# microsoft/timewarp

Hardware: AMD Instinct MI355X
Metric: MH-accepted samples/sec (whole node), alanine-dipeptide kernel_transformer_nvp (higher is better)
Workload: dtype f16x3 (split-fp16 operands, 3 MFMAs per fp32 product, fp32 accumulate)

## Files before the change

### timewarp_amd/csrc/tw_netblock_h3.hip

```cpp
#include <utility>
#include <vector>

#include "tw_common.h"

namespace tw {

typedef float f4 __attribute__((ext_vector_type(4)));
typedef _Float16 h8 __attribute__((ext_vector_type(8)));
typedef _Float16 h4 __attribute__((ext_vector_type(4)));
typedef unsigned u4 __attribute__((ext_vector_type(4)));
typedef unsigned u2 __attribute__((ext_vector_type(2)));

#define H3_NT 3
#define H3_FFN_SPLIT 4
#define H3_TOK (16 * H3_NT)
#define H3_XT 48
#define H3_XT_IMG 1536
#define H3_PAIR_BYTES 2048
#define H3_STAGE_PAIRS 4
#define H3_STAGE_TILE_BYTES 8192
#define H3_STAGE_BYTES 9216
#define H3_RING 5
#define H3_XT_BYTES (128 * H3_XT * 2)
#define H3_WAVE_LDS (2 * H3_XT_BYTES)
// ... 488 lines not shown
      for (int m = 0; m < V; ++m) row[m] = row[m] / den;
  }
  __syncthreads();
  char* out = sfrag + blockIdx.z * variant_bytes + blk * (int64_t)4 * H * ((int64_t)NG * nt * 2048);
  const bool paired = nt == H3N4_NT;
  for (int i = t; i < 4 * NG * nt * 64; i += nthr) {
    const int lane = i & 63, rest = i >> 6;
    const int jt = rest % nt, gi = (rest / nt) % NG, w = rest / (nt * NG);
    const int tq = 16 * nt * w + 16 * jt + (lane & 15);
    const int mq = tq / P, aq = tq - mq * P;
    const bool qok = mq < mpwg && aq < V;
    const float* row = E + (int64_t)(qok ? mq * V + aq : 0) * V;
    const int k0 = 16 * (win.w[w] / 32 + 2 * gi) + 8 * (lane >> 4);
    h8 hi, lo;
#pragma unroll
    for (int e = 0; e < 8; ++e) {
      const int tk = paired ? mq * P + 32 * gi + 4 * (lane >> 4) + (e < 4 ? e : e + 12) : k0 + e;
      const int ak = tk - mq * P;
      const float val = (qok && ak >= 0 && ak < V) ? row[ak] : 0.f;
      const _Float16 hh = (_Float16)val;
      hi[e] = hh;
      lo[e] = (_Float16)(val - (float)hh);
    }
    char* base = out + ((int64_t)(w * H + h) * (NG * nt) + (paired ? jt * NG + gi : gi * nt + jt)) * 2048;
    *(h8*)(base + lane * 16) = hi;
    *(h8*)(base + 1024 + lane * 16) = lo;
  }
}

struct H3Params {
  const char* packed;
  int64_t net_stride_bytes;
  int64_t stages;
  int64_t side_in2b, side_layers, side_layer_size, side_out2b, side_scales;
  const float* emb;
  const int32_t* types;
  const float* xc;
  const float* xv;
  const float* z_other;
  const char* sfrag;
  int sfrag_shared;
  int64_t sf_variant_bytes;
  int windowed;
  const float* rff;
  int d_rff;
  int win[4];
  float* out[2];
  float* dump;
  int64_t n_rows, n_cond;
  int V, mpw, nblocks;
  int ng;
  int P;
  int H, n_layers, ff_chunks, hid_chunks, d_emb;
  float eps;
  int net_sel;
  int debug;
  const uint8_t* masked;
  PrevCoupling prev;
};
__device__ __forceinline__ void h3_load_sf4(const char* p, u4 (&r)[16]) {
  asm volatile(
      "global_load_dwordx4 %0, %16, off\n\t"
      "global_load_dwordx4 %1, %16, off offset:1024\n\t"
      "global_load_dwordx4 %2, %16, off offset:2048\n\t"
      "global_load_dwordx4 %3, %16, off offset:3072\n\t"
      "global_load_dwordx4 %4, %17, off\n\t"
      "global_load_dwordx4 %5, %17, off offset:1024\n\t"
      "global_load_dwordx4 %6, %17, off offset:2048\n\t"
      "global_load_dwordx4 %7, %17, off offset:3072\n\t"
      "global_load_dwordx4 %8, %18, off\n\t"
      "global_load_dwordx4 %9, %18, off offset:1024\n\t"
      "global_load_dwordx4 %10, %18, off offset:2048\n\t"
      "global_load_dwordx4 %11, %18, off offset:3072\n\t"
      "global_load_dwordx4 %12, %19, off\n\t"
      "global_load_dwordx4 %13, %19, off offset:1024\n\t"
      "global_load_dwordx4 %14, %19, off offset:2048\n\t"
      "global_load_dwordx4 %15, %19, off offset:3072\n\t"
      "s_waitcnt vmcnt(0)"
      : "=&v"(r[0]), "=&v"(r[1]), "=&v"(r[2]), "=&v"(r[3]), "=&v"(r[4]), "=&v"(r[5]), "=&v"(r[6]), "=&v"(r[7]), "=&v"(r[8]),
        "=&v"(r[9]), "=&v"(r[10]), "=&v"(r[11]), "=&v"(r[12]), "=&v"(r[13]), "=&v"(r[14]), "=&v"(r[15])
      : "v"(p), "v"(p + H3N4_SF_BYTES), "v"(p + 2 * H3N4_SF_BYTES), "v"(p + 3 * H3N4_SF_BYTES)
      : "memory");
}

template <int NT>
struct BOp {
  h8 h[NT], l[NT];
};

__device__ __forceinline__ f4 mfma32(h8 a, h8 b, f4 c) { return __builtin_amdgcn_mfma_f32_16x16x32_f16(a, b, c, 0, 0, 0); }
__device__ __forceinline__ f4 mfma16(h4 a, h4 b, f4 c) { return __builtin_amdgcn_mfma_f32_16x16x16f16(a, b, c, 0, 0, 0); }

template <int NT>
__device__ __forceinline__ void mma3(const h8 ah, const h8 al, const BOp<NT>& b, f4 (&acc)[NT]) {
#pragma unroll
  for (int jt = 0; jt < NT; ++jt) acc[jt] = mfma32(ah, b.h[jt], acc[jt]);
#pragma unroll
  for (int jt = 0; jt < NT; ++jt) acc[jt] = mfma32(ah, b.l[jt], acc[jt]);
#pragma unroll
  for (int jt = 0; jt < NT; ++jt) acc[jt] = mfma32(al, b.h[jt], acc[jt]);
}

__device__ __forceinline__ void split_pair(float a, float b, unsigned& hi, unsigned& lo) {
  float ta, tb;
  asm("v_cvt_pk_f16_f32 %0, %4, %5\n\t"
      "v_fma_mix_f32 %2, %0, -1.0, %4 op_sel_hi:[1,0,0]\n\t"
// ... 58 lines not shown
      "global_load_dwordx4 %1, %12, off offset:1024\n\t"
      "global_load_dwordx2 %2, %13, off offset:2048\n\t"
      "global_load_dwordx2 %3, %13, off offset:2056\n\t"
      "global_load_dwordx4 %4, %14, off\n\t"
      "global_load_dwordx4 %5, %14, off offset:1024\n\t"
      "global_load_dwordx2 %6, %15, off offset:2048\n\t"
      "global_load_dwordx2 %7, %15, off offset:2056\n\t"
      "global_load_dwordx4 %8, %16, off\n\t"
      "global_load_dwordx4 %9, %16, off offset:1024\n\t"
      "global_load_dwordx2 %10, %17, off offset:2048\n\t"
      "global_load_dwordx2 %11, %17, off offset:2056\n\t"
      "s_waitcnt vmcnt(0)"
      : "=&v"(a[0]), "=&v"(b[0]), "=&v"(c[0]), "=&v"(d[0]), "=&v"(a[1]), "=&v"(b[1]), "=&v"(c[1]), "=&v"(d[1]),
        "=&v"(a[2]), "=&v"(b[2]), "=&v"(c[2]), "=&v"(d[2])
      : "v"(p16), "v"(p8), "v"(p16 + H3_SF_BYTES), "v"(p8 + H3_SF_BYTES), "v"(p16 + 2 * H3_SF_BYTES),
        "v"(p8 + 2 * H3_SF_BYTES)
      : "memory");
}



template <int NT>
__device__ __forceinline__ void h3_add_layernorm(f4 (&x)[8][NT], const f4 (&y)[8][NT], const float* lnw_lane,
                                                 const float* lnb_lane, float eps) {
  f4 w[8], b[8];
#pragma unroll
  for (int ft = 0; ft < 8; ++ft) {
    w[ft] = *(const f4*)(lnw_lane + 16 * ft);
    b[ft] = *(const f4*)(lnb_lane + 16 * ft);
  }
#pragma unroll
  for (int jt = 0; jt < NT; ++jt) {
    float s = 0.f;
#pragma unroll
    for (int ft = 0; ft < 8; ++ft) {
      x[ft][jt] = x[ft][jt] + y[ft][jt];
      s += (x[ft][jt][0] + x[ft][jt][1]) + (x[ft][jt][2] + x[ft][jt][3]);
    }
    const float mean = h3_xor_sum(s) * (1.f / 128.f);
    float q = 0.f;
#pragma unroll
    for (int ft = 0; ft < 8; ++ft) {
      x[ft][jt] = x[ft][jt] - mean;
      q += (x[ft][jt][0] * x[ft][jt][0] + x[ft][jt][1] * x[ft][jt][1]) +
           (x[ft][jt][2] * x[ft][jt][2] + x[ft][jt][3] * x[ft][jt][3]);
    }
    const float var = h3_xor_sum(q) * (1.f / 128.f);
    const float rstd = 1.0f / sqrtf(var + eps);
#pragma unroll
    for (int ft = 0; ft < 8; ++ft) x[ft][jt] = x[ft][jt] * rstd * w[ft] + b[ft];
  }
}

struct H3Pipe {
  const char* gnext;
  char* lds;
  int cur;
  int wave;
  int debug;
  int ring = H3_RING;

  __device__ __forceinline__ void fetch(int slot) {
    char* dst = lds + slot * H3_STAGE_BYTES;
#pragma unroll
    for (int i = 0; i < 2; ++i)
      __builtin_amdgcn_global_load_lds((const __attribute__((address_space(1))) void*)(gnext + wave * 2048 + i * 1024),
                                       (__attribute__((address_space(3))) void*)(dst + wave * 2048 + i * 1024), 16, 0, 0);
    if (wave == 0)
      __builtin_amdgcn_global_load_lds((const __attribute__((address_space(1))) void*)(gnext + H3_STAGE_TILE_BYTES),
                                       (__attribute__((address_space(3))) void*)(dst + H3_STAGE_TILE_BYTES), 16, 0, 0);
    gnext += H3_STAGE_BYTES;
  }
  __device__ __forceinline__ void start_issue() {
#pragma unroll
    for (int i = 0; i < H3_RING; ++i)
      if (i < ring) fetch(i);
    cur = 0;
  }
  __device__ __forceinline__ void start_wait() {
    asm volatile("s_waitcnt vmcnt(0)" ::: "memory");
    __builtin_amdgcn_s_barrier();
    asm volatile("" ::: "memory");
  }
  __device__ __forceinline__ const char* stage() const { return lds + cur * H3_STAGE_BYTES; }
  __device__ __forceinline__ void advance() {
    asm volatile("s_waitcnt vmcnt(0) lgkmcnt(0)" ::: "memory");
    if (!TW_EXPERIMENT(debug & TW_DEBUG_EXP_NO_BARRIERS)) __builtin_amdgcn_s_barrier();
    asm volatile("" ::: "memory");
    const int released = cur;
    cur = (cur + 1 == ring) ? 0 : cur + 1;
    if (!TW_EXPERIMENT(debug & TW_DEBUG_EXP_NO_WEIGHT_DMA)) fetch(released);
  }
};

struct H3Tiles {
  h8 t[2 * H3_STAGE_PAIRS];
  const char* base;
  __device__ __forceinline__ void rd(int p) {
    t[2 * p] = *(const h8*)(base + p * H3_PAIR_BYTES);
    t[2 * p + 1] = *(const h8*)(base + p * H3_PAIR_BYTES + 1024);
  }
  __device__ __forceinline__ void load(const char* st, int lane) {
    base = st + lane * 16;
    rd(0);
    rd(1);
    __builtin_amdgcn_sched_barrier(0);
// ... 114 lines not shown

template <int NT, bool ASM, bool DENSE = false, bool WIDE = false, bool RFF = false, bool ENC = false, bool H1 = false, bool NG6 = false>
__global__ void __launch_bounds__(256) __attribute__((amdgpu_waves_per_eu(1, 1)))
netblock_h3_kernel(const H3Params p) {
  extern __shared__ __attribute__((aligned(16))) char lds[];
  static_assert(!H1 || ENC || WIDE || (DENSE && ASM && !RFF) || (NT == 4 && ASM),
                "the single-MFMA variant exists as the encoder-stack build (<= 48 atoms), for the wide layout, and - MLP sections "
                "only, the softmax attention block stays in split form - for the dense model");
  static_assert(!WIDE || (ASM && !DENSE), "the wide layout exists for the asm build of the kernel-attention variant");
  static_assert(!NG6 || WIDE, "six-group windows belong to the wide layout");
  static_assert(!RFF || DENSE, "position features belong to the dense model");
  static_assert(!ENC || ASM, "the encoder-stack statement embeds the generated asm sections");
  static_assert(NT == 3 || (NT == 4 && !RFF && (!WIDE || (ENC && !NG6)) && (!DENSE || (ASM && !WIDE && !H1))),
                "64-token waves: the kernel-attention variant - one molecule of 49-64 atoms per wave, or (WIDE: the paired layout, "
                "encoder-stack statement only) one of 97-128 atoms per pair of waves; the dense softmax model on one molecule of "
                "49-64 atoms per wave: the encoder-stack statement (r06, tools/gen_h3_enc_asm.py --dense --nt=4), or the per-section "
                "build with its attention block compiled C++ (r05; activation dumps, section stamps)");
  constexpr int KIN = RFF ? 6 : 2;
  constexpr bool ASM_IO = ASM, ASM_ATT = ASM && !(DENSE && NT == 4);
  constexpr bool R6 = H3_R6(NT, DENSE, WIDE, RFF, ENC, H1);
  constexpr int RING = NT == 4 ? H3N4_RING : (R6 ? H3_RING + 1 : H3_RING);
  constexpr int XT_IMG = NT == 4 ? H3N4_XT_IMG : H3_XT_IMG;
  constexpr int SF_BYTES = NT == 4 ? H3N4_SF_BYTES : H3_SF_BYTES;
  constexpr int WAVE_LDS = NT == 4 ? H3N4_WAVE_LDS : (DENSE ? H3D_WAVE_LDS : (WIDE ? H3W_WAVE_LDS : H3_WAVE_LDS));
  constexpr int SIDE_LDS_OFFSET = NT == 4 ? H3N4_SIDE_LDS_OFFSET
                                          : (DENSE ? H3D_SIDE_LDS_OFFSET : (WIDE ? H3W_SIDE_LDS_OFFSET
                                                                                  : H3_SIDE_LDS_OFFSET + (R6 ? H3_STAGE_BYTES : 0)));
  constexpr int SIDE_CHUNKS = DENSE ? 5 : 3;
  const int wave = __builtin_amdgcn_readfirstlane(threadIdx.x >> 6);
  const int lane = threadIdx.x & 63;
  const int g = lane >> 4, i16 = lane & 15;

  int net, wg;
  if (p.net_sel < 0) {
    const int xcd = blockIdx.x & 7;
    net = xcd >> 2;
    wg = (blockIdx.x >> 3) * 4 + (xcd & 3);
  } else {
    net = p.net_sel;
    wg = blockIdx.x;
  }
  const int blk = wg * 4 + wave;
  const bool active = WIDE ? true : blk < p.nblocks;
  if (WIDE ? wg >= p.nblocks : wg * 4 >= p.nblocks) return;
  const int64_t row0 = (WIDE ? (int64_t)wg : (int64_t)blk) * p.mpw;
  const int slot0 = WIDE ? 16 * NT * wave : 0;

  const char* net_base = p.packed + (int64_t)net * p.net_stride_bytes;
  const float* side = (const float*)(net_base + p.stages * H3_STAGE_BYTES);
  const float* scales = side + p.side_scales;
  _Float16* xt_hi = (_Float16*)(lds + RING * H3_STAGE_BYTES + wave * WAVE_LDS);

  const unsigned long long t_kernel_top = (p.debug & TW_DEBUG_SECTION_STAMPS) ? __builtin_readcyclecounter() : 0ull;
  H3Pipe pipe;
  pipe.gnext = net_base + lane * 16;
  pipe.lds = lds;
  pipe.cur = 0;
  pipe.wave = wave;
  pipe.debug = p.debug;
  pipe.ring = RING;
  if constexpr (ENC && DENSE && NT == 3) {
    if (wave == 0) {
      const char* src = (const char*)(side + p.side_layers) + lane * 16;
      char* dst = lds + SIDE_LDS_OFFSET;
#pragma unroll
      for (int i = 0; i < SIDE_CHUNKS; ++i)
        __builtin_amdgcn_global_load_lds((const __attribute__((address_space(1))) void*)(src + i * 1024),
                                         (__attribute__((address_space(3))) void*)(dst + i * 1024), 16, 0, 0);
    }
  }
  pipe.start_issue();

  const float sc_in2 = scales[1], sc_out2 = scales[2 + 3 * p.n_layers + 1];
  f4 bb_in2[8];
#pragma unroll
  for (int ot = 0; ot < 8; ++ot) bb_in2[ot] = *(const f4*)(side + p.side_in2b + 4 * g + 16 * ot);
  const f4 bb_out2 = *(const f4*)(side + p.side_out2b + 4 * g);

  int64_t tok_row[NT];
  int64_t tok_cond[NT];
  int tok_atom[NT];
  const unsigned inv_v = (65536u + (unsigned)p.P - 1u) / (unsigned)p.P;
  const bool cond_shared = p.n_cond == 1, cond_per_row = p.n_cond >= p.n_rows;
#pragma unroll
  for (int jt = 0; jt < NT; ++jt) {
    const int t = slot0 + 16 * jt + i16;
    const int q = (int)(((unsigned)t * inv_v) >> 16);
    const int64_t n = row0 + q;
    const int atom = t - q * p.P;
    const bool ok = active && q < p.mpw && n < p.n_rows && atom < p.V;
    tok_row[jt] = ok ? n : -1;
    tok_cond[jt] = !ok || cond_shared ? 0 : (cond_per_row ? n : n % p.n_cond);
    tok_atom[jt] = ok ? atom : 0;
  }
  float zo[NT][3];
  {
    float part[NT];
    bool bad = false;
#pragma unroll
    for (int jt = 0; jt < NT; ++jt) {
      const int64_t n = tok_row[jt];
      part[jt] = 0.f;
#pragma unroll
      for (int k = 0; k < 3; ++k) zo[jt][k] = 0.f;
      if (n < 0) continue;
      const int64_t idx = (n * p.V + tok_atom[jt]) * 3;
      if (p.prev.s_raw) {
        float ld = 0.f;
#pragma unroll
        for (int k = 0; k < 3; ++k) {
          const float sr = p.prev.s_raw[idx + k], shift = p.prev.t[idx + k];
          const float scale = expf(sr);
          bad |= !(isfinite(sr) && isfinite(shift));
          const float z = p.prev.z_in[idx + k];
          zo[jt][k] = p.prev.reverse ? (z - shift) / scale : z * scale + shift;
          ld += logf(scale);
        }
        part[jt] = p.masked[tok_cond[jt] * p.V + tok_atom[jt]] ? 0.f : ld;
        if (net == 0 && g == 0) {
#pragma unroll
          for (int k = 0; k < 3; ++k) p.prev.z_out[idx + k] = zo[jt][k];
        }
      } else {
#pragma unroll
        for (int k = 0; k < 3; ++k) zo[jt][k] = p.z_other[idx + k];
      }
    }
    if constexpr (WIDE) {
      if (p.prev.s_raw) {
        float* scr = (float*)(lds + RING * H3_STAGE_BYTES);
        if (net == 0) {
          if (bad) atomicOr(p.prev.nonfinite, 1);
          if (g == 0) {
#pragma unroll
            for (int jt = 0; jt < NT; ++jt) scr[slot0 + 16 * jt + i16] = part[jt];
          }
        }
        asm volatile("s_waitcnt lgkmcnt(0)" ::: "memory");
        __builtin_amdgcn_s_barrier();
        if (net == 0 && wave == 0 && lane < p.mpw) {
          const int64_t n = row0 + lane;
          if (n < p.n_rows) {
            float acc = 0.f;
            for (int a = 0; a < p.V; ++a) acc += scr[lane * p.P + a];
            p.prev.delta_logp[n] -= p.prev.reverse ? -acc : acc;
          }
        }
        asm volatile("s_waitcnt lgkmcnt(0)" ::: "memory");
        __builtin_amdgcn_s_barrier();
      }
    } else
    if (p.prev.s_raw && net == 0) {
      if (bad) atomicOr(p.prev.nonfinite, 1);
      float* scr = (float*)xt_hi;
      if (g == 0) {
#pragma unroll
        for (int jt = 0; jt < NT; ++jt) scr[16 * jt + i16] = part[jt];
      }
      if (lane < p.mpw) {
        const int64_t n = (int64_t)blk * p.mpw + lane;
        if (active && n < p.n_rows) {
          float acc = 0.f;
          for (int a = 0; a < p.V; ++a) acc += scr[lane * p.V + a];
          p.prev.delta_logp[n] -= p.prev.reverse ? -acc : acc;
        }
      }
    }
  }
  const unsigned long long t_pro1 = (p.debug & TW_DEBUG_SECTION_STAMPS) ? __builtin_readcyclecounter() : 0ull;
  BOp<NT> u[KIN];
  const bool std_input = !RFF && p.d_emb == 32;
  if (std_input) {
#pragma unroll
    for (int jt = 0; jt < NT; ++jt) {
      const int64_t n = tok_row[jt];
      const int64_t ca = n < 0 ? 0 : tok_cond[jt] * p.V + tok_atom[jt];
      const int ty = n < 0 ? 0 : p.types[ca];
      const float* er = p.emb + ty * 32 + 4 * g;
      f4 e0, e1, m;
#pragma unroll
      for (int r = 0; r < 4; ++r) { e0[r] = er[r]; e1[r] = er[16 + r]; }
      const float c0 = p.xc[ca * 3], c1 = p.xc[ca * 3 + 1], c2 = p.xc[ca * 3 + 2];
      const float v0 = p.xv[ca * 3], v1 = p.xv[ca * 3 + 1], v2 = p.xv[ca * 3 + 2];
      m[0] = g == 0 ? c0 : g == 1 ? v1 : g == 2 ? zo[jt][2] : 0.f;
      m[1] = g == 0 ? c1 : g == 1 ? v2 : 0.f;
      m[2] = g == 0 ? c2 : g == 1 ? zo[jt][0] : 0.f;
      m[3] = g == 0 ? v0 : g == 1 ? zo[jt][1] : 0.f;
      if (n < 0) e0 = e1 = m = (f4){0.f, 0.f, 0.f, 0.f};
      split8(e0, e1, u[0].h[jt], u[0].l[jt]);
      split8(m, (f4){0.f, 0.f, 0.f, 0.f}, u[1].h[jt], u[1].l[jt]);
    }
  } else
#pragma unroll
  for (int jt = 0; jt < NT; ++jt) {
    const int64_t n = tok_row[jt];
    const int64_t c = tok_cond[jt];
    const int a = tok_atom[jt];
    const int ty = n < 0 ? 0 : p.types[c * p.V + a];
#pragma unroll
    for (int ks = 0; ks < KIN; ++ks)
#pragma unroll
      for (int e = 0; e < 8; ++e) {
        const int f = 32 * ks + 16 * (e / 4) + 4 * g + (e % 4);
        float val = 0.f;
        if (n >= 0) {
          if (f < p.d_emb) val = p.emb[ty * p.d_emb + f];
          else if (f < p.d_emb + 3) val = p.xc[(c * p.V + a) * 3 + (f - p.d_emb)];
          else if (f < p.d_emb + 6) val = p.xv[(c * p.V + a) * 3 + (f - p.d_emb - 3)];
          else if (f < p.d_emb + 9) val = zo[jt][f - p.d_emb - 6];
          else if (RFF && f < p.d_emb + 9 + p.d_rff) {
            const float* px = p.xc + (c * p.V + a) * 3;
            const int nvec = p.d_rff / 2;
            const int j = f - p.d_emb - 9;
            const int col = j % nvec;
            const float ip = px[0] * p.rff[0 * nvec + col] + px[1] * p.rff[1 * nvec + col] + px[2] * p.rff[2 * nvec + col];
            val = sqrtf(1.0f / nvec) * (j < nvec ? cosf(ip) : sinf(ip));
          }
        }
        const _Float16 hi = (_Float16)val;
        u[ks].h[jt][e] = hi;
        u[ks].l[jt][e] = (_Float16)(val - (float)hi);
      }
  }
  asm volatile("" : "+v"(u[0].h[0]), "+v"(u[1].h[0]));
  const unsigned long long t_pro2 = (p.debug & TW_DEBUG_SECTION_STAMPS) ? __builtin_readcyclecounter() : 0ull;
  if constexpr (!ENC)
    for (int i = lane; i < WAVE_LDS / 16; i += 64) ((f4*)xt_hi)[i] = (f4){0.f, 0.f, 0.f, 0.f};

  const unsigned long long t_pro3 = (p.debug & TW_DEBUG_SECTION_STAMPS) ? __builtin_readcyclecounter() : 0ull;
  pipe.start_wait();

  auto dump_x = [&](const f4 (&x)[8][NT], int stage) {
    if (!p.dump) return;
    float* d = p.dump + (int64_t)stage * p.n_rows * p.V * 128;
#pragma unroll
    for (int jt = 0; jt < NT; ++jt) {
      if (tok_row[jt] < 0) continue;
      float* row = d + (tok_row[jt] * p.V + tok_atom[jt]) * 128;
#pragma unroll
      for (int ft = 0; ft < 8; ++ft) *(f4*)(row + 16 * ft + 4 * g) = x[ft][jt];
    }
  };

  auto stamp = [&](int idx) {
    if ((p.debug & TW_DEBUG_SECTION_STAMPS) && p.dump && blockIdx.x == 0 && wave == 0 && lane == 0)
      ((unsigned long long*)p.dump)[idx] = __builtin_readcyclecounter();
  };
  stamp(0);
  if ((p.debug & TW_DEBUG_SECTION_STAMPS) && p.dump && blockIdx.x == 0 && wave == 0 && lane == 0) {
    ((unsigned long long*)p.dump)[60] = t_kernel_top;
    ((unsigned long long*)p.dump)[61] = t_pro1;
    ((unsigned long long*)p.dump)[62] = t_pro2;
    ((unsigned long long*)p.dump)[63] = t_pro3;
  }

  f4 x[8][NT];
  {
#pragma unroll
    for (int ot = 0; ot < 8; ++ot)
#pragma unroll
      for (int jt = 0; jt < NT; ++jt) x[ot][jt] = (f4){0.f, 0.f, 0.f, 0.f};
    if constexpr (ASM_IO && !RFF) {
      char* priv = (char*)xt_hi;
#pragma unroll
      for (int ks = 0; ks < 2; ++ks)
#pragma unroll
        for (int jt = 0; jt < NT; ++jt) {
          *(h8*)(priv + ((ks * NT + jt) * 2) * 1024 + lane * 16) = u[ks].h[jt];
          *(h8*)(priv + ((ks * NT + jt) * 2 + 1) * 1024 + lane * 16) = u[ks].l[jt];
        }
      int cur = __builtin_amdgcn_readfirstlane(pipe.cur);
      const char* gn = pipe.gnext;
      const unsigned ring = (unsigned)(uintptr_t)(const __attribute__((address_space(3))) char*)lds;
      const unsigned priv_lds = (unsigned)(uintptr_t)(const __attribute__((address_space(3))) char*)priv;
      const int chunks = __builtin_amdgcn_readfirstlane(p.hid_chunks);
      if constexpr (NT == 4 && H1) {
        asm volatile(
#include "tw_h1n4_in_asm.inc"
            : [cur] "+&s"(cur), [gn] "+&v"(gn)
            : [ring] "s"(ring), [wave] "s"(wave), [priv] "s"(priv_lds), [chunks] "s"(chunks)
            :
#include "tw_h1n4_in_clobbers.inc"
        );
      } else if constexpr (NT == 4) {
        asm volatile(
#include "tw_h3n4_in_asm.inc"
            : [cur] "+&s"(cur), [gn] "+&v"(gn)
            : [ring] "s"(ring), [wave] "s"(wave), [priv] "s"(priv_lds), [chunks] "s"(chunks)
            :
#include "tw_h3n4_in_clobbers.inc"
        );
      } else if constexpr (R6) {
        asm volatile(
#include "tw_h1r_in_asm.inc"
            : [cur] "+&s"(cur), [gn] "+&v"(gn)
            : [ring] "s"(ring), [wave] "s"(wave), [priv] "s"(priv_lds), [chunks] "s"(chunks)
            :
#include "tw_h1r_in_clobbers.inc"
        );
      } else if constexpr (H1) {
        asm volatile(
#include "tw_h1_in_asm.inc"
            : [cur] "+&s"(cur), [gn] "+&v"(gn)
            : [ring] "s"(ring), [wave] "s"(wave), [priv] "s"(priv_lds), [chunks] "s"(chunks)
            :
#include "tw_h1_in_clobbers.inc"
// ... 1384 lines not shown
    if (d.variant == 0 ? (layout == 0 ? h3_narrow_ok(d, n_atoms) : layout == 1 ? h3_wide_ok(n_atoms) : h3_nt4_ok(d, n_atoms, false))
                       : (layout == 0 ? !h3_nt4_ok(d, n_atoms, false) : layout == 2 && h3_nt4_ok(d, n_atoms, false))) {
      const int64_t x = h3_ws(d, n_rows, n_atoms, nullptr, false, layout).bytes;
      if (x > b) b = x;
    }
  return b;
}

static int h3_launch(const FlowArgs& a, const RawLayout& L, const FusedGeom& fg, int c, int net_sel, const float* z_other,
                     const char* sfrag, int64_t sf_variant_bytes, bool shared, float* s_out, float* t_out, float* dump,
                     const PrevCoupling& prev = PrevCoupling{}, bool dry = false) {
  const tw_flow_desc& d = *a.desc;
  const bool h1 = a.h1 != 0;
  const H3Geom g = h3_geom(d, h1);
  H3Params p;
  p.packed = (const char*)a.packed + (int64_t)(c * 2) * g.net_stride_bytes;
  p.net_stride_bytes = g.net_stride_bytes;
  p.stages = g.stages;
  p.side_in2b = g.side_in2b;
  p.side_layers = g.side_layers;
  p.side_layer_size = g.side_layer_size;
  p.side_out2b = g.side_out2b;
  p.side_scales = g.side_scales;
  p.emb = a.raw + L.emb;
  p.types = a.atom_types;
  p.xc = a.x_coords;
  p.xv = a.x_velocs;
  p.z_other = z_other;
  p.sfrag = sfrag;
  p.sfrag_shared = shared ? 1 : 0;
  p.sf_variant_bytes = sf_variant_bytes;
  H3Wide wd{};
  const bool wide = h3_wide_choice(d, a.n_atoms, a.n_rows, h1);
  if (wide) h3_wide_geom(a.n_atoms, &wd);
  p.d_rff = d.variant == 1 ? d.d_rff : 0;
  p.rff = p.d_rff > 0 ? a.raw + L.chain + (int64_t)c * L.coupling_size + L.rff : nullptr;
  p.windowed = (!wide && h3_windowed(fg, a.n_atoms)) ? 1 : 0;
  for (int i = 0; i < 4; ++i) p.win[i] = wide ? wd.win[i] : 0;
  p.out[0] = s_out;
  p.out[1] = t_out;
  p.dump = dump;
  p.n_rows = a.n_rows;
  p.n_cond = a.n_cond;
  p.V = a.n_atoms;
  p.P = wide ? wd.stride : a.n_atoms;
  p.ng = wide ? wd.ng : 0;
  p.mpw = fg.mpw;
  p.nblocks = (int)((a.n_rows + fg.mpw - 1) / fg.mpw);
  p.H = d.n_heads;
  p.n_layers = d.n_layers;
  p.ff_chunks = g.ff_chunks;
  p.hid_chunks = g.hid_chunks;
  p.d_emb = d.d_emb;
  p.eps = d.ln_eps;
  p.net_sel = net_sel;
  p.debug = g_debug_flags;
  p.masked = a.masked;
  p.prev = prev;
  const int wgs_per_net = wide ? p.nblocks : (p.nblocks + 3) / 4;
  unsigned grid = net_sel < 0 ? 8u * (unsigned)((wgs_per_net + 3) / 4) : (unsigned)wgs_per_net;
  int prc;
  if (!dry && (prc = profile_mark(a.stream, true))) return prc;
#define H3_STR2(...) #__VA_ARGS__
#define H3_STR(...) H3_STR2(__VA_ARGS__)
#define H3_LAUNCH(LDS, ...)                                                                                        \
  do {                                                                                                             \
    note_netblock_kernel("tw::netblock_h3_kernel<" H3_STR(__VA_ARGS__) ">");                                       \
    if (dry) return TW_OK;           \
    static LdsLimit lim;                                                                                           \
    if ((prc = lim.ensure((const void*)netblock_h3_kernel<__VA_ARGS__>, (int)(LDS)))) return prc;                  \
    hipLaunchKernelGGL((netblock_h3_kernel<__VA_ARGS__>), dim3(grid), dim3(256), (LDS), a.stream, p);              \
  } while (0)
  const bool per_section = ((dump != nullptr || (g_debug_flags & (TW_DEBUG_DUMP_ATTENTION | TW_DEBUG_SECTION_STAMPS | TW_DEBUG_PER_SECTION))) &&
                            !(g_debug_flags & TW_DEBUG_ENC_WITH_DUMPS)) ||
                           d.n_layers < 1;
  const bool cpp = (g_debug_flags & TW_DEBUG_COMPILED_CPP) != 0;
  if (wide && wd.nt == H3N4_NT) {
    TW_REQUIRE(d.variant == 0 && !per_section && !cpp, "paired 64-token layout: the encoder-stack statement only");
    if (h1) H3_LAUNCH(H3N4_LDS_BYTES, 4, true, false, true, false, true, true, false);
    else H3_LAUNCH(H3N4_LDS_BYTES, 4, true, false, true, false, true, false, false);
  } else if (!wide && fg.nt == H3N4_NT && d.variant == 1) {
    TW_REQUIRE(!h1 && d.d_rff == 0 && !cpp, "dense model on 64-token waves: the split-fp16 build without position features");
    if (per_section) H3_LAUNCH(H3D4_LDS_BYTES, 4, true, true, false, false, false, false, false);
    else H3_LAUNCH(H3D4_LDS_BYTES, 4, true, true, false, false, true, false, false);
  } else if (!wide && fg.nt == H3N4_NT) {
    TW_REQUIRE(d.variant == 0, "64-token waves: kernel attention");
    if (h1 && per_section) H3_LAUNCH(H3N4_LDS_BYTES, 4, true, false, false, false, false, true, false);
    else if (h1) H3_LAUNCH(H3N4_LDS_BYTES, 4, true, false, false, false, true, true, false);
    else if (cpp) H3_LAUNCH(H3N4_LDS_BYTES, 4, false, false, false, false, false, false, false);
    else if (per_section) H3_LAUNCH(H3N4_LDS_BYTES, 4, true, false, false, false, false, false, false);
    else H3_LAUNCH(H3N4_LDS_BYTES, 4, true, false, false, false, true, false, false);
  } else if (h1) {
    TW_REQUIRE(h1_supported(d, a.n_atoms) && d.n_layers >= 1, "single-MFMA path: unsupported configuration");
    if (d.variant == 1 && d.d_rff > 0) {
      TW_REQUIRE(!per_section, "single-MFMA path with position features: the encoder-stack statement only");
      H3_LAUNCH(H3D_ENC_LDS_BYTES, 3, true, true, false, true, true, true, false);
    } else if (d.variant == 1) {
      if (per_section) H3_LAUNCH(H3D_LDS_BYTES, 3, true, true, false, false, false, true, false);
      else H3_LAUNCH(H3D_ENC_LDS_BYTES, 3, true, true, false, false, true, true, false);
    } else if (wide) {
      if (per_section && wd.ng == H3W_NG6) H3_LAUNCH(H3W_LDS_BYTES, 3, true, false, true, false, false, true, true);
      else if (per_section) H3_LAUNCH(H3W_LDS_BYTES, 3, true, false, true, false, false, true, false);
      else if (wd.ng == H3W_NG6) H3_LAUNCH(H3W_LDS_BYTES, 3, true, false, true, false, true, true, true);
      else H3_LAUNCH(H3W_LDS_BYTES, 3, true, false, true, false, true, true, false);
    } else {
      TW_REQUIRE(dump == nullptr || (g_debug_flags & TW_DEBUG_SECTION_STAMPS), "single-MFMA path: no activation dumps (section stamps only)");
// ... 315 lines not shown
```

Measured before the change: 158.8.

## Batch prologue global loads up front and defer coupling-layer stores past pipeline wait

Restructures the kernel prologue so all per-token global loads (types, xc/xv, z, s_raw/t, masked, embeddings, old delta_logp) are issued together before any dependent math, instead of interleaved load-compute chains. The z_out and delta_logp stores are moved after pipe.start_wait so they do not sit between the weight-pipeline issue and its wait. The per-row log-det sum uses an 8-wide ordered gather to expose load parallelism. It also adds extra debug cycle stamps. In exchange it raises register pressure, and it issues loads for invalid tokens (clamped to index 0).

```diff
diff --git a/timewarp_amd/csrc/tw_netblock_h3.hip b/timewarp_amd/csrc/tw_netblock_h3.hip
--- a/timewarp_amd/csrc/tw_netblock_h3.hip
+++ b/timewarp_amd/csrc/tw_netblock_h3.hip
@@ -728,6 +728,18 @@
   }
 }
 
+__device__ __forceinline__ float h3_ordered_sum(const float* v, int n) {
+  float acc = 0.f;
+  for (int a0 = 0; a0 < n; a0 += 8) {
+    float x[8];
+#pragma unroll
+    for (int i = 0; i < 8; ++i) x[i] = v[a0 + i < n ? a0 + i : n - 1];
+#pragma unroll
+    for (int i = 0; i < 8; ++i) acc = a0 + i < n ? acc + x[i] : acc;
+  }
+  return acc;
+}
+
 struct H3Pipe {
   const char* gnext;
   char* lds;
@@ -973,6 +985,7 @@
   for (int ot = 0; ot < 8; ++ot) bb_in2[ot] = *(const f4*)(side + p.side_in2b + 4 * g + 16 * ot);
   const f4 bb_out2 = *(const f4*)(side + p.side_out2b + 4 * g);
 
+  const unsigned long long t_pro_top = (p.debug & TW_DEBUG_SECTION_STAMPS) ? __builtin_readcyclecounter() : 0ull;
   int64_t tok_row[NT];
   int64_t tok_cond[NT];
   int tok_atom[NT];
@@ -989,41 +1002,87 @@
     tok_cond[jt] = !ok || cond_shared ? 0 : (cond_per_row ? n : n % p.n_cond);
     tok_atom[jt] = ok ? atom : 0;
   }
+  const bool has_prev = p.prev.s_raw != nullptr;
+  const bool std_input = !RFF && p.d_emb == 32;
+  int64_t tok_ca[NT], tok_idx[NT];
+#pragma unroll
+  for (int jt = 0; jt < NT; ++jt) {
+    tok_ca[jt] = tok_cond[jt] * p.V + tok_atom[jt];
+    tok_idx[jt] = tok_row[jt] < 0 ? 0 : (tok_row[jt] * p.V + tok_atom[jt]) * 3;
+  }
+  int tok_type[NT];
+  float cx[NT][3], cv[NT][3];
+#pragma unroll
+  for (int jt = 0; jt < NT; ++jt) tok_type[jt] = p.types[tok_ca[jt]];
+#pragma unroll
+  for (int jt = 0; jt < NT; ++jt)
+#pragma unroll
+    for (int k = 0; k < 3; ++k) {
+      cx[jt][k] = p.xc[tok_ca[jt] * 3 + k];
+      cv[jt][k] = p.xv[tok_ca[jt] * 3 + k];
+    }
   float zo[NT][3];
+  float pv_s[NT][3], pv_t[NT][3];
+  uint8_t pv_masked[NT];
+  const int64_t ld_row = row0 + lane;
+  const bool ld_lane = has_prev && net == 0 && lane < p.mpw && ld_row < p.n_rows && (WIDE ? wave == 0 : active);
+  float ld_old = 0.f, ld_new = 0.f;
+  {
+    const float* zsrc = has_prev ? p.prev.z_in : p.z_other;
+#pragma unroll
+    for (int jt = 0; jt < NT; ++jt)
+#pragma unroll
+      for (int k = 0; k < 3; ++k) zo[jt][k] = zsrc[tok_idx[jt] + k];
+  }
+  if (has_prev) {
+#pragma unroll
+    for (int jt = 0; jt < NT; ++jt) {
+#pragma unroll
+      for (int k = 0; k < 3; ++k) {
+        pv_s[jt][k] = p.prev.s_raw[tok_idx[jt] + k];
+        pv_t[jt][k] = p.prev.t[tok_idx[jt] + k];
+      }
+      pv_masked[jt] = p.masked[tok_ca[jt]];
+    }
+    if (ld_lane) ld_old = p.prev.delta_logp[ld_row];
+  }
+  const unsigned long long t_pro_ld = (p.debug & TW_DEBUG_SECTION_STAMPS) ? __builtin_readcyclecounter() : 0ull;
+  f4 emb0[NT], emb1[NT];
+#pragma unroll
+  for (int jt = 0; jt < NT; ++jt) {
+    const float* er = (std_input ? p.emb + tok_type[jt] * 32 : side + p.side_in2b) + 4 * g;
+#pragma unroll
+    for (int r = 0; r < 4; ++r) { emb0[jt][r] = er[r]; emb1[jt][r] = er[16 + r]; }
+  }
+  unsigned long long t_pro_cpl = 0ull;
   {
     float part[NT];
     bool bad = false;
 #pragma unroll
     for (int jt = 0; jt < NT; ++jt) {
-      const int64_t n = tok_row[jt];
       part[jt] = 0.f;
-#pragma unroll
-      for (int k = 0; k < 3; ++k) zo[jt][k] = 0.f;
-      if (n < 0) continue;
-      const int64_t idx = (n * p.V + tok_atom[jt]) * 3;
-      if (p.prev.s_raw) {
+      if (has_prev) {
         float ld = 0.f;
 #pragma unroll
         for (int k = 0; k < 3; ++k) {
-          const float sr = p.prev.s_raw[idx + k], shift = p.prev.t[idx + k];
+          const float sr = pv_s[jt][k], shift = pv_t[jt][k];
           const float scale = expf(sr);
-          bad |= !(isfinite(sr) && isfinite(shift));
-          const float z = p.prev.z_in[idx + k];
+          bad |= (tok_row[jt] >= 0) & !(isfinite(sr) & isfinite(shift));
+          const float z = zo[jt][k];
           zo[jt][k] = p.prev.reverse ? (z - shift) / scale : z * scale + shift;
           ld += logf(scale);
         }
-        part[jt] = p.masked[tok_cond[jt] * p.V + tok_atom[jt]] ? 0.f : ld;
-        if (net == 0 && g == 0) {
-#pragma unroll
-          for (int k = 0; k < 3; ++k) p.prev.z_out[idx + k] = zo[jt][k];
-        }
-      } else {
-#pragma unroll
-        for (int k = 0; k < 3; ++k) zo[jt][k] = p.z_other[idx + k];
-      }
-    }
+        part[jt] = pv_masked[jt] ? 0.f : ld;
+      }
+      if (tok_row[jt] < 0) {
+        part[jt] = 0.f;
+#pragma unroll
+        for (int k = 0; k < 3; ++k) zo[jt][k] = 0.f;
+      }
+    }
+    t_pro_cpl = (p.debug & TW_DEBUG_SECTION_STAMPS) ? __builtin_readcyclecounter() : 0ull;
     if constexpr (WIDE) {
-      if (p.prev.s_raw) {
+      if (has_prev) {
         float* scr = (float*)(lds + RING * H3_STAGE_BYTES);
         if (net == 0) {
           if (bad) atomicOr(p.prev.nonfinite, 1);
@@ -1034,55 +1093,40 @@
         }
         asm volatile("s_waitcnt lgkmcnt(0)" ::: "memory");
         __builtin_amdgcn_s_barrier();
-        if (net == 0 && wave == 0 && lane < p.mpw) {
-          const int64_t n = row0 + lane;
-          if (n < p.n_rows) {
-            float acc = 0.f;
-            for (int a = 0; a < p.V; ++a) acc += scr[lane * p.P + a];
-            p.prev.delta_logp[n] -= p.prev.reverse ? -acc : acc;
-          }
+        if (ld_lane) {
+          const float acc = h3_ordered_sum(scr + lane * p.P, p.V);
+          ld_new = ld_old - (p.prev.reverse ? -acc : acc);
         }
         asm volatile("s_waitcnt lgkmcnt(0)" ::: "memory");
         __builtin_amdgcn_s_barrier();
       }
     } else
-    if (p.prev.s_raw && net == 0) {
+    if (has_prev && net == 0) {
       if (bad) atomicOr(p.prev.nonfinite, 1);
       float* scr = (float*)xt_hi;
       if (g == 0) {
 #pragma unroll
         for (int jt = 0; jt < NT; ++jt) scr[16 * jt + i16] = part[jt];
       }
-      if (lane < p.mpw) {
-        const int64_t n = (int64_t)blk * p.mpw + lane;
-        if (active && n < p.n_rows) {
-          float acc = 0.f;
-          for (int a = 0; a < p.V; ++a) acc += scr[lane * p.V + a];
-          p.prev.delta_logp[n] -= p.prev.reverse ? -acc : acc;
-        }
+      if (ld_lane) {
+        const float acc = h3_ordered_sum(scr + lane * p.V, p.V);
+        ld_new = ld_old - (p.prev.reverse ? -acc : acc);
       }
     }
   }
   const unsigned long long t_pro1 = (p.debug & TW_DEBUG_SECTION_STAMPS) ? __builtin_readcyclecounter() : 0ull;
   BOp<NT> u[KIN];
-  const bool std_input = !RFF && p.d_emb == 32;
   if (std_input) {
 #pragma unroll
     for (int jt = 0; jt < NT; ++jt) {
-      const int64_t n = tok_row[jt];
-      const int64_t ca = n < 0 ? 0 : tok_cond[jt] * p.V + tok_atom[jt];
-      const int ty = n < 0 ? 0 : p.types[ca];
-      const float* er = p.emb + ty * 32 + 4 * g;
-      f4 e0, e1, m;
-#pragma unroll
-      for (int r = 0; r < 4; ++r) { e0[r] = er[r]; e1[r] = er[16 + r]; }
-      const float c0 = p.xc[ca * 3], c1 = p.xc[ca * 3 + 1], c2 = p.xc[ca * 3 + 2];
-      const float v0 = p.xv[ca * 3], v1 = p.xv[ca * 3 + 1], v2 = p.xv[ca * 3 + 2];
+      f4 e0 = emb0[jt], e1 = emb1[jt], m;
+      const float c0 = cx[jt][0], c1 = cx[jt][1], c2 = cx[jt][2];
+      const float v0 = cv[jt][0], v1 = cv[jt][1], v2 = cv[jt][2];
       m[0] = g == 0 ? c0 : g == 1 ? v1 : g == 2 ? zo[jt][2] : 0.f;
       m[1] = g == 0 ? c1 : g == 1 ? v2 : 0.f;
       m[2] = g == 0 ? c2 : g == 1 ? zo[jt][0] : 0.f;
       m[3] = g == 0 ? v0 : g == 1 ? zo[jt][1] : 0.f;
-      if (n < 0) e0 = e1 = m = (f4){0.f, 0.f, 0.f, 0.f};
+      if (tok_row[jt] < 0) e0 = e1 = m = (f4){0.f, 0.f, 0.f, 0.f};
       split8(e0, e1, u[0].h[jt], u[0].l[jt]);
       split8(m, (f4){0.f, 0.f, 0.f, 0.f}, u[1].h[jt], u[1].l[jt]);
     }
@@ -1125,6 +1169,17 @@
 
   const unsigned long long t_pro3 = (p.debug & TW_DEBUG_SECTION_STAMPS) ? __builtin_readcyclecounter() : 0ull;
   pipe.start_wait();
+  if (has_prev && net == 0) {
+    if (g == 0) {
+#pragma unroll
+      for (int jt = 0; jt < NT; ++jt) {
+        if (tok_row[jt] < 0) continue;
+#pragma unroll
+        for (int k = 0; k < 3; ++k) p.prev.z_out[tok_idx[jt] + k] = zo[jt][k];
+      }
+    }
+    if (ld_lane) p.prev.delta_logp[ld_row] = ld_new;
+  }
 
   auto dump_x = [&](const f4 (&x)[8][NT], int stage) {
     if (!p.dump) return;
@@ -1148,6 +1203,9 @@
     ((unsigned long long*)p.dump)[61] = t_pro1;
     ((unsigned long long*)p.dump)[62] = t_pro2;
     ((unsigned long long*)p.dump)[63] = t_pro3;
+    ((unsigned long long*)p.dump)[64] = t_pro_top;
+    ((unsigned long long*)p.dump)[65] = t_pro_ld;
+    ((unsigned long long*)p.dump)[66] = t_pro_cpl;
   }
 
   f4 x[8][NT];
```

After: 159.5, median of 6. No clear change (+0.4%).

## Hoist prologue global loads ahead of weight pipe and defer log-det reduction

Applied to the files above, without the earlier changes.

Moves all per-token global loads (previous coupling s/t/z, types, mask, xc, xv, delta_logp) to the very top of the kernel, before the weight-stream pipe starts, so their latency overlaps with pipe setup. It preloads up to eight embedding rows into registers and selects among them instead of doing a dependent gather per token. The delta_logp reduction and its barriers move after pipe.start_wait, using an unrolled row sum, and the LDS scratch is re-zeroed for the decoder path. This raises register pressure and reorders the LDS scratch use, which could hurt occupancy or correctness if the scratch overlaps pipe data.

```diff
diff --git a/timewarp_amd/csrc/tw_netblock_h3.hip b/timewarp_amd/csrc/tw_netblock_h3.hip
--- a/timewarp_amd/csrc/tw_netblock_h3.hip
+++ b/timewarp_amd/csrc/tw_netblock_h3.hip
@@ -564,6 +564,7 @@
   int ng;
   int P;
   int H, n_layers, ff_chunks, hid_chunks, d_emb;
+  int n_types;
   float eps;
   int net_sel;
   int debug;
@@ -948,6 +949,63 @@
   _Float16* xt_hi = (_Float16*)(lds + RING * H3_STAGE_BYTES + wave * WAVE_LDS);
 
   const unsigned long long t_kernel_top = (p.debug & TW_DEBUG_SECTION_STAMPS) ? __builtin_readcyclecounter() : 0ull;
+  int64_t tok_row[NT];
+  int64_t tok_cond[NT];
+  int tok_atom[NT];
+  const unsigned inv_v = (65536u + (unsigned)p.P - 1u) / (unsigned)p.P;
+  const bool cond_shared = p.n_cond == 1, cond_per_row = p.n_cond >= p.n_rows;
+#pragma unroll
+  for (int jt = 0; jt < NT; ++jt) {
+    const int t = slot0 + 16 * jt + i16;
+    const int q = (int)(((unsigned)t * inv_v) >> 16);
+    const int64_t n = row0 + q;
+    const int atom = t - q * p.P;
+    const bool ok = active && q < p.mpw && n < p.n_rows && atom < p.V;
+    tok_row[jt] = ok ? n : -1;
+    tok_cond[jt] = !ok || cond_shared ? 0 : (cond_per_row ? n : n % p.n_cond);
+    tok_atom[jt] = ok ? atom : 0;
+  }
+  typedef float f3u __attribute__((ext_vector_type(3), aligned(4)));
+  typedef float f4u __attribute__((ext_vector_type(4), aligned(4)));
+  const bool pending = p.prev.s_raw != nullptr;
+  const float* cs_src = pending ? p.prev.s_raw : p.z_other;
+  const float* ct_src = pending ? p.prev.t : p.z_other;
+  const float* cz_src = pending ? p.prev.z_in : p.z_other;
+  f3u ld_s[NT], ld_t[NT], ld_z[NT], ld_xc[NT], ld_xv[NT];
+  int ld_ty[NT];
+  uint8_t ld_mk[NT];
+  int64_t tok_idx[NT];
+#pragma unroll
+  for (int jt = 0; jt < NT; ++jt) {
+    const int64_t n = tok_row[jt];
+    tok_idx[jt] = n < 0 ? 0 : (n * p.V + tok_atom[jt]) * 3;
+    const int64_t ca = tok_cond[jt] * p.V + tok_atom[jt];
+    ld_s[jt] = *(const f3u*)(cs_src + tok_idx[jt]);
+    ld_t[jt] = *(const f3u*)(ct_src + tok_idx[jt]);
+    ld_z[jt] = *(const f3u*)(cz_src + tok_idx[jt]);
+    ld_ty[jt] = p.types[ca];
+    ld_mk[jt] = p.masked[ca];
+    ld_xc[jt] = *(const f3u*)(p.xc + ca * 3);
+    ld_xv[jt] = *(const f3u*)(p.xv + ca * 3);
+  }
+  constexpr int H3_EMB_ROWS = 8;
+  const bool std_input = !RFF && p.d_emb == 32;
+  const bool emb_select = std_input && p.n_types <= H3_EMB_ROWS;
+  f4 emb0[H3_EMB_ROWS], emb1[H3_EMB_ROWS];
+  if (emb_select) {
+#pragma unroll
+    for (int r = 0; r < H3_EMB_ROWS; ++r) {
+      const float* er = p.emb + (r < p.n_types ? r : p.n_types - 1) * 32 + 4 * g;
+      emb0[r] = *(const f4u*)er;
+      emb1[r] = *(const f4u*)(er + 16);
+    }
+  }
+  const int64_t red_row = row0 + lane;
+  const bool red_lane = pending && net == 0 && (WIDE ? wave == 0 : active) && lane < p.mpw && red_row < p.n_rows;
+  float red_logp = 0.f;
+  if (pending) red_logp = p.prev.delta_logp[red_lane ? red_row : 0];
+  __builtin_amdgcn_sched_barrier(0);
+
   H3Pipe pipe;
   pipe.gnext = net_base + lane * 16;
   pipe.lds = lds;
@@ -973,111 +1031,62 @@
   for (int ot = 0; ot < 8; ++ot) bb_in2[ot] = *(const f4*)(side + p.side_in2b + 4 * g + 16 * ot);
   const f4 bb_out2 = *(const f4*)(side + p.side_out2b + 4 * g);
 
-  int64_t tok_row[NT];
-  int64_t tok_cond[NT];
-  int tok_atom[NT];
-  const unsigned inv_v = (65536u + (unsigned)p.P - 1u) / (unsigned)p.P;
-  const bool cond_shared = p.n_cond == 1, cond_per_row = p.n_cond >= p.n_rows;
+  float zo[NT][3];
+  float part[NT];
+  bool bad = false;
 #pragma unroll
   for (int jt = 0; jt < NT; ++jt) {
-    const int t = slot0 + 16 * jt + i16;
-    const int q = (int)(((unsigned)t * inv_v) >> 16);
-    const int64_t n = row0 + q;
-    const int atom = t - q * p.P;
-    const bool ok = active && q < p.mpw && n < p.n_rows && atom < p.V;
-    tok_row[jt] = ok ? n : -1;
-    tok_cond[jt] = !ok || cond_shared ? 0 : (cond_per_row ? n : n % p.n_cond);
-    tok_atom[jt] = ok ? atom : 0;
-  }
-  float zo[NT][3];
-  {
-    float part[NT];
-    bool bad = false;
+    const bool ok = tok_row[jt] >= 0;
+    part[jt] = 0.f;
+    if (pending) {
+      float ld = 0.f;
+#pragma unroll
+      for (int k = 0; k < 3; ++k) {
+        const float sr = ld_s[jt][k], shift = ld_t[jt][k];
+        const float scale = expf(sr);
+        bad |= ok && !(isfinite(sr) && isfinite(shift));
+        const float z = ld_z[jt][k];
+        zo[jt][k] = p.prev.reverse ? (z - shift) / scale : z * scale + shift;
+        ld += logf(scale);
+      }
+      part[jt] = ld_mk[jt] ? 0.f : ld;
+      if (ok && net == 0 && g == 0) {
+#pragma unroll
+        for (int k = 0; k < 3; ++k) p.prev.z_out[tok_idx[jt] + k] = zo[jt][k];
+      }
+    } else {
+#pragma unroll
+      for (int k = 0; k < 3; ++k) zo[jt][k] = ld_z[jt][k];
+    }
+    if (!ok) {
+      part[jt] = 0.f;
+#pragma unroll
+      for (int k = 0; k < 3; ++k) zo[jt][k] = 0.f;
+    }
+  }
+  const unsigned long long t_pro1 = (p.debug & TW_DEBUG_SECTION_STAMPS) ? __builtin_readcyclecounter() : 0ull;
+  BOp<NT> u[KIN];
+  if (std_input) {
 #pragma unroll
     for (int jt = 0; jt < NT; ++jt) {
       const int64_t n = tok_row[jt];
-      part[jt] = 0.f;
-#pragma unroll
-      for (int k = 0; k < 3; ++k) zo[jt][k] = 0.f;
-      if (n < 0) continue;
-      const int64_t idx = (n * p.V + tok_atom[jt]) * 3;
-      if (p.prev.s_raw) {
-        float ld = 0.f;
-#pragma unroll
-        for (int k = 0; k < 3; ++k) {
-          const float sr = p.prev.s_raw[idx + k], shift = p.prev.t[idx + k];
-          const float scale = expf(sr);
-          bad |= !(isfinite(sr) && isfinite(shift));
-          const float z = p.prev.z_in[idx + k];
-          zo[jt][k] = p.prev.reverse ? (z - shift) / scale : z * scale + shift;
-          ld += logf(scale);
-        }
-        part[jt] = p.masked[tok_cond[jt] * p.V + tok_atom[jt]] ? 0.f : ld;
-        if (net == 0 && g == 0) {
-#pragma unroll
-          for (int k = 0; k < 3; ++k) p.prev.z_out[idx + k] = zo[jt][k];
+      const int ty = n < 0 ? 0 : ld_ty[jt];
+      f4 e0, e1, m;
+      if (emb_select) {
+        e0 = emb0[0];
+        e1 = emb1[0];
+#pragma unroll
+        for (int r = 1; r < H3_EMB_ROWS; ++r) {
+          e0 = ty == r ? emb0[r] : e0;
+          e1 = ty == r ? emb1[r] : e1;
         }
       } else {
-#pragma unroll
-        for (int k = 0; k < 3; ++k) zo[jt][k] = p.z_other[idx + k];
-      }
-    }
-    if constexpr (WIDE) {
-      if (p.prev.s_raw) {
-        float* scr = (float*)(lds + RING * H3_STAGE_BYTES);
-        if (net == 0) {
-          if (bad) atomicOr(p.prev.nonfinite, 1);
-          if (g == 0) {
-#pragma unroll
-            for (int jt = 0; jt < NT; ++jt) scr[slot0 + 16 * jt + i16] = part[jt];
-          }
-        }
-        asm volatile("s_waitcnt lgkmcnt(0)" ::: "memory");
-        __builtin_amdgcn_s_barrier();
-        if (net == 0 && wave == 0 && lane < p.mpw) {
-          const int64_t n = row0 + lane;
-          if (n < p.n_rows) {
-            float acc = 0.f;
-            for (int a = 0; a < p.V; ++a) acc += scr[lane * p.P + a];
-            p.prev.delta_logp[n] -= p.prev.reverse ? -acc : acc;
-          }
-        }
-        asm volatile("s_waitcnt lgkmcnt(0)" ::: "memory");
-        __builtin_amdgcn_s_barrier();
-      }
-    } else
-    if (p.prev.s_raw && net == 0) {
-      if (bad) atomicOr(p.prev.nonfinite, 1);
-      float* scr = (float*)xt_hi;
-      if (g == 0) {
-#pragma unroll
-        for (int jt = 0; jt < NT; ++jt) scr[16 * jt + i16] = part[jt];
-      }
-      if (lane < p.mpw) {
-        const int64_t n = (int64_t)blk * p.mpw + lane;
-        if (active && n < p.n_rows) {
-          float acc = 0.f;
-          for (int a = 0; a < p.V; ++a) acc += scr[lane * p.V + a];
-          p.prev.delta_logp[n] -= p.prev.reverse ? -acc : acc;
-        }
-      }
-    }
-  }
-  const unsigned long long t_pro1 = (p.debug & TW_DEBUG_SECTION_STAMPS) ? __builtin_readcyclecounter() : 0ull;
-  BOp<NT> u[KIN];
-  const bool std_input = !RFF && p.d_emb == 32;
-  if (std_input) {
-#pragma unroll
-    for (int jt = 0; jt < NT; ++jt) {
-      const int64_t n = tok_row[jt];
-      const int64_t ca = n < 0 ? 0 : tok_cond[jt] * p.V + tok_atom[jt];
-      const int ty = n < 0 ? 0 : p.types[ca];
-      const float* er = p.emb + ty * 32 + 4 * g;
-      f4 e0, e1, m;
-#pragma unroll
-      for (int r = 0; r < 4; ++r) { e0[r] = er[r]; e1[r] = er[16 + r]; }
-      const float c0 = p.xc[ca * 3], c1 = p.xc[ca * 3 + 1], c2 = p.xc[ca * 3 + 2];
-      const float v0 = p.xv[ca * 3], v1 = p.xv[ca * 3 + 1], v2 = p.xv[ca * 3 + 2];
+        const float* er = p.emb + ty * 32 + 4 * g;
+#pragma unroll
+        for (int r = 0; r < 4; ++r) { e0[r] = er[r]; e1[r] = er[16 + r]; }
+      }
+      const float c0 = ld_xc[jt][0], c1 = ld_xc[jt][1], c2 = ld_xc[jt][2];
+      const float v0 = ld_xv[jt][0], v1 = ld_xv[jt][1], v2 = ld_xv[jt][2];
       m[0] = g == 0 ? c0 : g == 1 ? v1 : g == 2 ? zo[jt][2] : 0.f;
       m[1] = g == 0 ? c1 : g == 1 ? v2 : 0.f;
       m[2] = g == 0 ? c2 : g == 1 ? zo[jt][0] : 0.f;
@@ -1092,7 +1101,7 @@
     const int64_t n = tok_row[jt];
     const int64_t c = tok_cond[jt];
     const int a = tok_atom[jt];
-    const int ty = n < 0 ? 0 : p.types[c * p.V + a];
+    const int ty = n < 0 ? 0 : ld_ty[jt];
 #pragma unroll
     for (int ks = 0; ks < KIN; ++ks)
 #pragma unroll
@@ -1125,8 +1134,64 @@
 
   const unsigned long long t_pro3 = (p.debug & TW_DEBUG_SECTION_STAMPS) ? __builtin_readcyclecounter() : 0ull;
   pipe.start_wait();
-
-  auto dump_x = [&](const f4 (&x)[8][NT], int stage) {
+  const unsigned long long t_pro4 = (p.debug & TW_DEBUG_SECTION_STAMPS) ? __builtin_readcyclecounter() : 0ull;
+
+  if (pending) {
+    auto row_sum = [&](const float* row) {
+      float acc = 0.f;
+      for (int a0 = 0; a0 < p.V; a0 += 8) {
+        float v[8];
+#pragma unroll
+        for (int i = 0; i < 8; ++i) v[i] = row[a0 + i < p.V ? a0 + i : p.V - 1];
+#pragma unroll
+        for (int i = 0; i < 8; ++i) acc = a0 + i < p.V ? acc + v[i] : acc;
+      }
+      return acc;
+    };
+    if constexpr (WIDE) {
+      float* scr = (float*)(lds + RING * H3_STAGE_BYTES);
+      if (net == 0) {
+        if (bad) atomicOr(p.prev.nonfinite, 1);
+        if (g == 0) {
+#pragma unroll
+          for (int jt = 0; jt < NT; ++jt) scr[slot0 + 16 * jt + i16] = part[jt];
+        }
+      }
+      asm volatile("s_waitcnt lgkmcnt(0)" ::: "memory");
+      __builtin_amdgcn_s_barrier();
+      if (red_lane) {
+        const float acc = row_sum(scr + lane * p.P);
+        p.prev.delta_logp[red_row] = red_logp - (p.prev.reverse ? -acc : acc);
+      }
+      asm volatile("s_waitcnt lgkmcnt(0)" ::: "memory");
+      __builtin_amdgcn_s_barrier();
+      if constexpr (!ENC) {
+        if (net == 0 && g == 0) {
+#pragma unroll
+          for (int jt = 0; jt < NT; ++jt) scr[slot0 + 16 * jt + i16] = 0.f;
+        }
+      }
+    } else if (net == 0) {
+      if (bad) atomicOr(p.prev.nonfinite, 1);
+      float* scr = (float*)xt_hi;
+      if (g == 0) {
+#pragma unroll
+        for (int jt = 0; jt < NT; ++jt) scr[16 * jt + i16] = part[jt];
+      }
+      if (red_lane) {
+        const float acc = row_sum(scr + lane * p.V);
+        p.prev.delta_logp[red_row] = red_logp - (p.prev.reverse ? -acc : acc);
+      }
+      if constexpr (!ENC) {
+        if (g == 0) {
+#pragma unroll
+          for (int jt = 0; jt < NT; ++jt) scr[16 * jt + i16] = 0.f;
+        }
+      }
+    }
+  }
+
+  auto dump_x =[&](const f4 (&x)[8][NT], int stage) {
     if (!p.dump) return;
     float* d = p.dump + (int64_t)stage * p.n_rows * p.V * 128;
 #pragma unroll
@@ -1148,6 +1213,7 @@
     ((unsigned long long*)p.dump)[61] = t_pro1;
     ((unsigned long long*)p.dump)[62] = t_pro2;
     ((unsigned long long*)p.dump)[63] = t_pro3;
+    ((unsigned long long*)p.dump)[67] = t_pro4;
   }
 
   f4 x[8][NT];
@@ -2638,6 +2704,7 @@
   p.ff_chunks = g.ff_chunks;
   p.hid_chunks = g.hid_chunks;
   p.d_emb = d.d_emb;
+  p.n_types = d.n_elements;
   p.eps = d.ln_eps;
   p.net_sel = net_sel;
   p.debug = g_debug_flags;
```

Measured after the change: 158.0 before, 158.4 after, median of 6. About the same (+0.3%).
